# graphdeco-inria/editable-gaussian-reflections

Hardware: AMD Instinct MI355X
Metric: Mrays/s fwd+bwd @1080p, 1M Gaussians (higher is better)
Workload: dtype f32; 1 GPU; BASELINE config C: synthetic dense-init room+spheres cloud, HEADLINE variant = init (literal dense-init opacity 0.1 (config.py:44): Kc ~ 22 per ray, bounces mostly die), N=1000000, 1920x1080, one training iteration: export + update_bvh + forward + backward + grad import, num_bounces=2, jitter on, reference default config; variant=init, gaussians=1000000, width=1920, height=1080, parallelism=image tiles x1 + 1 all-reduce of the launch's [22N] gradients, team_help=product default (on)

## Files before the change

### editable-gaussian-reflections_amd/csrc/backward_chain.hpp

```cpp
#pragma once

constexpr int BOUNCE_QUEUE_FLOATS = 25 * EGR_WAVE;
static_assert(EGR_GT_STRIDE * EGR_GT_SLOTS >= BOUNCE_QUEUE_FLOATS, "the bounce queues must fit into the table");

template <int TEAM> struct BwdWave {
    int lane, wv;
    uint32_t *gt_keys;
    float *gt_vals;
    uint32_t *gt_claim;
    float4 *stage;
    BwdTeamShared<TEAM> &bteam;
    uint4 *bitems;
    float *bdl;
    float *bray;
    float exp_power;
    int num_bounces;
    float view_size;
    uint32_t bepoch;
    bool table_dirty;
};

struct BwdDiag {
    EGR_TIMES(unsigned long long bw_t0 = 0ull, bw_t1 = 0ull; uint32_t bw_rows0 = 0u;)
};
// ... 8 lines not shown

template <bool PRIMARY, bool BATCH, int TEAM>
EGR_DI RayGrads output_gradients(const DeviceView &v, const BwdWave<TEAM> &W, const ChainTask &task, const TaskGeom &tg, const StateRef &S, const int step,
                                 const uint32_t steps_done, const uint32_t nhits) {
    RayGrads g{mk3(0, 0, 0), mk3(0, 0, 0), mk3(0, 0, 0), 0.0f, 0.0f, mk3(0, 0, 0), mk3(0, 0, 1), mk3(0, 0, 0), mk3(0, 0, 0), mk3(0, 0, 0), 0.0f, 0.0f, 0.0f};
    if (nhits > 0) {
        const uint32_t pid = tg.pixel_id;
        const float third = 1.0f / 3.0f;
        if constexpr (PRIMARY) {
            f3 o_rgb = S.ld3(SF(0, S_RGB)), o_n = S.ld3(SF(0, S_NORMAL)), o_f0 = S.ld3(SF(0, S_F0));
            float o_depth = S.ld(SF(0, S_DEPTH)), o_rough = S.ld(SF(0, S_ROUGH));
            if constexpr (BATCH) {
                const size_t P = v.num_pixels;
                const uint32_t bframe = task.bframe;
                auto tgt = [&](int b, uint32_t ch, uint32_t c) { const float *p = v.batch_targets[b]; return p ? p[((size_t)bframe * ch + c) * P + pid] : 0.0f; };
                g.dL_rgb = mk3(third * sign1(o_rgb.x - tgt(0, 3, 0)), third * sign1(o_rgb.y - tgt(0, 3, 1)), third * sign1(o_rgb.z - tgt(0, 3, 2))) * *v.cfg.loss_weight_diffuse;
                g.dL_depth = sign1(o_depth - tgt(2, 1, 0)) * *v.cfg.loss_weight_depth;
                g.dL_n = mk3(third * sign1(o_n.x - tgt(3, 3, 0)), third * sign1(o_n.y - tgt(3, 3, 1)), third * sign1(o_n.z - tgt(3, 3, 2))) * *v.cfg.loss_weight_normal;
                g.dL_f0 = mk3(third * sign1(o_f0.x - tgt(5, 3, 0)), third * sign1(o_f0.y - tgt(5, 3, 1)), third * sign1(o_f0.z - tgt(5, 3, 2))) * *v.cfg.loss_weight_f0;
                g.dL_rough = sign1(o_rough - tgt(4, 1, 0)) * *v.cfg.loss_weight_roughness;
            } else {
                const bool planes = v.target_planes != 0u;
                const size_t cs = planes ? (size_t)v.num_pixels : (size_t)1;
                auto tgt = [&](int b, uint32_t ch, uint32_t c) { const float *p = v.batch_targets[b]; return p ? p[(size_t)pid * (planes ? 1u : ch) + c * cs] : 0.0f; };
                g.dL_rgb = mk3(third * sign1(o_rgb.x - tgt(0, 3, 0)), third * sign1(o_rgb.y - tgt(0, 3, 1)), third * sign1(o_rgb.z - tgt(0, 3, 2))) * *v.cfg.loss_weight_diffuse;
                g.dL_depth = sign1(o_depth - tgt(2, 1, 0)) * *v.cfg.loss_weight_depth;
                g.dL_n = mk3(third * sign1(o_n.x - tgt(3, 3, 0)), third * sign1(o_n.y - tgt(3, 3, 1)), third * sign1(o_n.z - tgt(3, 3, 2))) * *v.cfg.loss_weight_normal;
                g.dL_f0 = mk3(third * sign1(o_f0.x - tgt(5, 3, 0)), third * sign1(o_f0.y - tgt(5, 3, 1)), third * sign1(o_f0.z - tgt(5, 3, 2))) * *v.cfg.loss_weight_f0;
                g.dL_rough = sign1(o_rough - tgt(4, 1, 0)) * *v.cfg.loss_weight_roughness;
            }
            const PrimaryRay p = primary_ray<BATCH>(v, tg, task, W.view_size);
            g.ro = p.ro, g.rd = p.rd;
        } else {
            f3 spec = mk3(0, 0, 0);
            for (int j = 1; j < W.num_bounces + 1; j++)
                if ((uint32_t)j < steps_done) spec = spec + S.ld3(SF(j, S_RGB));
            f3 t_spec;
            if constexpr (BATCH) {
                const float *p = v.batch_targets[1];
                const size_t P = v.num_pixels, q = (size_t)task.bframe * 3 * P + pid;
                t_spec = p ? mk3(p[q], p[q + P], p[q + 2 * P]) : mk3(0, 0, 0);
            } else {
                const float *p = v.batch_targets[1];
                const size_t q = (size_t)pid * (v.target_planes ? 1u : 3u), cs = v.target_planes ? (size_t)v.num_pixels : (size_t)1;
                t_spec = p ? mk3(p[q], p[q + cs], p[q + 2 * cs]) : mk3(0, 0, 0);
            }
            float down = powf(1.0f - S.ld(SF(step - 1, S_ROUGH)), EGR_ROUGHNESS_DOWNWEIGHT_GRAD_POWER);
            g.dL_rgb = (mk3(third * sign1(spec.x - t_spec.x), third * sign1(spec.y - t_spec.y), third * sign1(spec.z - t_spec.z)) *
                        *v.cfg.loss_weight_specular) * down;
            g.dL_rgb = g.dL_rgb * S.ld3(SF(step - 1, S_THR));
            g.ro = S.ld3(SF(step - 1, S_NEXT_O));
            g.rd = S.ld3(SF(step - 1, S_NEXT_D));
        }
        g.rem_rgb = S.ld3(SF(step, S_REM_RGB)), g.rem_n = S.ld3(SF(step, S_REM_NORMAL)), g.rem_f0 = S.ld3(SF(step, S_REM_F0));
        g.rem_depth = S.ld(SF(step, S_REM_DEPTH)), g.rem_rough = S.ld(SF(step, S_REM_ROUGH));
        g.T_minus_Ttot = S.ld(SF(step, S_T)) - S.ld(SF(step, S_TTOT));
    }
    return g;
}

template <int TEAM> EGR_DI uint32_t bounce_hits(const DeviceView &v, BwdWave<TEAM> &W, const RayGrads &g, uint32_t blk, const uint32_t nhits, const uint32_t max_hits) {
    const int lane = W.lane, wv = W.wv;
    const float exp_power = W.exp_power;
    BwdTeamShared<TEAM> &bteam = W.bteam;
    uint4 *const bitems = W.bitems;
    float *const bdl = W.bdl, *const bray = W.bray;
    float4 *const stage = W.stage;
    const f3 dL_rgb = g.dL_rgb, ro = g.ro, rd = g.rd, rem_rgb = g.rem_rgb;
    const float T_minus_Ttot = g.T_minus_Ttot;
    uint32_t records = 0u;
    W.table_dirty = true;
    bdl[lane] = dL_rgb.x, bdl[EGR_WAVE + lane] = dL_rgb.y, bdl[2 * EGR_WAVE + lane] = dL_rgb.z;
    bray[lane] = ro.x, bray[EGR_WAVE + lane] = ro.y, bray[2 * EGR_WAVE + lane] = ro.z, bray[3 * EGR_WAVE + lane] = rd.x, bray[4 * EGR_WAVE + lane] = rd.y, bray[5 * EGR_WAVE + lane] = rd.z;
    f3 prev_rgb = mk3(0, 0, 0), w_rgb = mk3(0, 0, 0);
    const uint32_t nblocks = (max_hits + EGR_HIT_BLOCK_ROWS - 1) / EGR_HIT_BLOCK_ROWS;
    EGR_BWD_SYNC();
    for (uint32_t b = nblocks; b-- > 0;) {
        const float4 *rows = v.hit_arena + (size_t)blk * (EGR_HIT_BLOCK_ROWS + 1) * EGR_WAVE;
        for (int chunk = EGR_HIT_BLOCK_ROWS / 4 - 1; chunk >= 0; chunk--) {
            uint32_t nitems = 0u;
            float4 rec4[4], a04[4];
#pragma unroll
            for (int r4 = 0; r4 < 4; r4++) rec4[r4] = rows[(size_t)(1 + 4 * chunk + r4) * EGR_WAVE + lane];
#pragma unroll
            for (int r4 = 0; r4 < 4; r4++) a04[r4] = v.app[2 * ((b * EGR_HIT_BLOCK_ROWS + (uint32_t)(4 * chunk + r4)) < nhits ? f2u(rec4[r4].x) : 0u)];
#pragma unroll
            for (int r4 = 3; r4 >= 0; r4--) {
                const int row = 4 * chunk + r4;
                const uint32_t it = b * EGR_HIT_BLOCK_ROWS + (uint32_t)row;
                const bool act = it < nhits;
                float dL_dalpha = 0.0f, weight = 0.0f;
                uint32_t pos = 0u;
                if (act) {
                    const float4 rec = rec4[r4];
                    pos = f2u(rec.x);
                    const float alpha = rec.z, transmittance = rec.w;
                    weight = (float)((double)transmittance / (1.0 - (double)alpha) * (double)alpha);
                    const float4 a0 = a04[r4];
                    const f3 g_rgb = mk3(a0.x, a0.y, a0.z);
                    w_rgb = w_rgb + (g_rgb - prev_rgb) * transmittance;
                    prev_rgb = g_rgb;
                    const float one_m_alpha = 1.0f - alpha, r1ma = egr_rcp_refined(one_m_alpha);
                    const float tmp1 = egr_div_rn(1.0f, one_m_alpha, r1ma);
                    dL_dalpha += dot(w_rgb * tmp1, dL_rgb);
                    const float tmp2 = -egr_div_rn(T_minus_Ttot, one_m_alpha, r1ma);
                    dL_dalpha += tmp2 * dot(rem_rgb, dL_rgb);
                }
                const unsigned long long am = __ballot(act);
                if (act) bitems[nitems + __builtin_amdgcn_mbcnt_hi((uint32_t)(am >> 32), __builtin_amdgcn_mbcnt_lo((uint32_t)am, 0u))] = make_uint4((uint32_t)lane, f2u(dL_dalpha), pos, f2u(weight));
                nitems += (uint32_t)__popcll(am);
            }
            if (nitems == 0u) continue;
            EGR_BWD_SYNC();
            const uint32_t nbatch = (nitems + (uint32_t)EGR_WAVE - 1u) / (uint32_t)EGR_WAVE;
            if constexpr (TEAM > 1) {
                if (lane == 0) {
                    lds_poke(&bteam.finished[wv], 0u);
                    lds_poke(&bteam.nitems[wv], nitems);
                    W.bepoch = (W.bepoch + 1u) & 0xFFFu;
                    lds_poke(&bteam.ticket[wv], (W.bepoch << 20) | (nbatch << 10));
                }
                for (;;) {
                    uint32_t tk = 0u;
                    if (lane == 0) tk = atomicAdd(&bteam.ticket[wv], 1u);
                    tk = uniform_u32(tk);
                    const uint32_t bi = tk & 0x3FFu;
                    if (bi >= nbatch) break;
                    records += bounce_batch(v, exp_power, bitems, bdl, bray, bi * (uint32_t)EGR_WAVE, nitems, stage, lane);
                    if (lane == 0) atomicAdd(&bteam.finished[wv], 1u);
                }
                while (uniform_u32(lds_peek(&bteam.finished[wv])) < nbatch) __builtin_amdgcn_s_sleep(1);
            } else {
                for (uint32_t bi = 0; bi < nbatch; bi++) records += bounce_batch(v, exp_power, bitems, bdl, bray, bi * (uint32_t)EGR_WAVE, nitems, stage, lane);
            }
            EGR_BWD_SYNC();
        }
        blk = f2u(rows[0].x);
    }
    return records;
}

template <int TEAM> EGR_DI uint32_t primary_hits(const DeviceView &v, BwdWave<TEAM> &W, const RayGrads &g, uint32_t blk, const uint32_t nhits, const uint32_t max_hits) {
    const int lane = W.lane;
    uint32_t *const gt_keys = W.gt_keys, *const gt_claim = W.gt_claim;
    float *const gt_vals = W.gt_vals;
    float4 *const stage = W.stage;
    const f3 dL_rgb = g.dL_rgb, dL_n = g.dL_n, dL_f0 = g.dL_f0, ro = g.ro, rd = g.rd, rem_rgb = g.rem_rgb, rem_n = g.rem_n, rem_f0 = g.rem_f0;
    const float dL_depth = g.dL_depth, dL_rough = g.dL_rough, rem_depth = g.rem_depth, rem_rough = g.rem_rough, T_minus_Ttot = g.T_minus_Ttot;
    uint32_t records = 0u;
    f3 prev_rgb = mk3(0, 0, 0), w_rgb = mk3(0, 0, 0), prev_n = mk3(0, 0, 0), w_n = mk3(0, 0, 0), prev_f0 = mk3(0, 0, 0), w_f0 = mk3(0, 0, 0);
    float prev_rough = 0, w_rough = 0, prev_depth = 0, w_depth = 0;
    const uint32_t nblocks = (max_hits + EGR_HIT_BLOCK_ROWS - 1) / EGR_HIT_BLOCK_ROWS;
    EGR_STATS(unsigned long long bt_math = 0ull, bt_table = 0ull, bt_wide = 0ull, bt_rows = 0ull;)
    for (uint32_t b = nblocks; b-- > 0;) {
        const float4 *rows = v.hit_arena + (size_t)blk * (EGR_HIT_BLOCK_ROWS + 1) * EGR_WAVE;
        int pf_row = -1;
        float4 rec_pf = make_float4(0.f, 0.f, 0.f, 0.f);
        for (int row = EGR_HIT_BLOCK_ROWS - 1; row >= 0; row--) {
            const uint32_t it = b * EGR_HIT_BLOCK_ROWS + (uint32_t)row;
            if (it >= max_hits) continue;
            bool direct = false, want = false;
            uint32_t dpos = 0;
            float gx[EGR_GT_COMPS];
            EGR_STATS(const unsigned long long bt0 = __builtin_amdgcn_s_memtime(); unsigned long long bt1 = bt0; bt_rows++;)
            float4 rec_cur = rec_pf;
            const bool have_pf = pf_row == row;
            if (row > 0) {
                if (it <= nhits) rec_pf = rows[(size_t)row * EGR_WAVE + lane];
                pf_row = row - 1;
            }
            if (!have_pf) {
                if (it < nhits) rec_cur = rows[(size_t)(1 + row) * EGR_WAVE + lane];
#if defined(__HIP_DEVICE_COMPILE__)
                asm volatile("" ::"v"(rec_cur.x), "v"(rec_cur.y), "v"(rec_cur.z), "v"(rec_cur.w));
#endif
            }
            if (it < nhits) {
                const float4 rec = rec_cur;
                const uint32_t pos = f2u(rec.x);
                const float distance = rec.y, alpha = rec.z, transmittance = rec.w;
                const float4 a0 = v.app[2 * pos], a1 = v.app[2 * pos + 1], a2 = v.inst_w[4 * pos + 3];
                const f3 g_rgb = mk3(a0.x, a0.y, a0.z);
                const float weight = (float)((double)transmittance / (1.0 - (double)alpha) * (double)alpha);
                f3 d_rgb = (dL_rgb * weight);
                f3 d_n = dL_n * weight, d_f0 = dL_f0 * weight;
                float d_rough = dL_rough * weight;

                w_rgb = w_rgb + (g_rgb - prev_rgb) * transmittance;
                prev_rgb = g_rgb;
                {
                    f3 g_n = mk3(a0.w, a1.x, a1.y), g_f0 = mk3(a1.z, a1.w, a2.x);
                    w_n = w_n + (g_n - prev_n) * transmittance;
                    prev_n = g_n;
                    w_f0 = w_f0 + (g_f0 - prev_f0) * transmittance;
                    prev_f0 = g_f0;
                    w_rough += (a2.y - prev_rough) * transmittance;
                    prev_rough = a2.y;
                    w_depth += (distance - prev_depth) * transmittance;
                    prev_depth = distance;
                }
                float dL_dalpha = 0.0f;
                const float one_m_alpha = 1.0f - alpha, r1ma = egr_rcp_refined(one_m_alpha);
                const float tmp1 = egr_div_rn(1.0f, one_m_alpha, r1ma);
                dL_dalpha += dot(w_rgb * tmp1, dL_rgb);
                dL_dalpha += dot(w_n * tmp1, dL_n);
                dL_dalpha += dot(w_f0 * tmp1, dL_f0);
                dL_dalpha += (w_rough * tmp1) * dL_rough;
                dL_dalpha += (w_depth * tmp1) * dL_depth;
                const float tmp2 = -egr_div_rn(T_minus_Ttot, one_m_alpha, r1ma);
                dL_dalpha += tmp2 * dot(rem_rgb, dL_rgb);
                dL_dalpha += tmp2 * dot(rem_n, dL_n);
                dL_dalpha += tmp2 * dot(rem_f0, dL_f0);
                dL_dalpha += tmp2 * (rem_rough * dL_rough);
                dL_dalpha += tmp2 * (rem_depth * dL_depth);

                hit_geometry_fn(v, W.exp_power, pos, a2, ro, rd, dL_dalpha, gx);
                gx[PC_RGB] = d_rgb.x, gx[PC_RGB + 1] = d_rgb.y, gx[PC_RGB + 2] = d_rgb.z, gx[PC_WEIGHT] = weight;
                gx[PC_NORMAL] = d_n.x, gx[PC_NORMAL + 1] = d_n.y, gx[PC_NORMAL + 2] = d_n.z;
                gx[PC_F0] = d_f0.x, gx[PC_F0 + 1] = d_f0.y, gx[PC_F0 + 2] = d_f0.z, gx[PC_ROUGH] = d_rough;
                EGR_STATS(bt1 = __builtin_amdgcn_s_memtime();)
                dpos = pos;
                want = primary_presum(pos, gx, lane);
            }
            direct = primary_table_add(v, want, dpos, gx, gt_keys, gt_vals, gt_claim, stage, lane, records);
            EGR_STATS(const unsigned long long bt2 = __builtin_amdgcn_s_memtime(); bt_math += bt1 - bt0; bt_table += bt2 - bt1;)
            if (__ballot(direct) != 0ull) {
                float lo[EGR_REC0_COMPS], hi[EGR_REC1_COMPS];
#pragma unroll
                for (int c = 0; c < EGR_REC0_COMPS; c++) lo[c] = gx[c];
#pragma unroll
                for (int c = 0; c < EGR_REC1_COMPS; c++) hi[c] = gx[EGR_REC0_COMPS + c];
                wide_add_wave<EGR_REC0_CELL>(v, direct, dpos, lo, stage);
                wide_add_wave<EGR_REC1_CELL>(v, direct, dpos, hi, stage);
                records += 2u * (uint32_t)__popcll(__ballot(direct));
            }
            EGR_STATS(bt_wide += __builtin_amdgcn_s_memtime() - bt2;)
        }
        blk = f2u(rows[0].x);
    }
    EGR_STATS(const unsigned long long bt3 = __builtin_amdgcn_s_memtime();)
    records += grad_table_flush(v, gt_keys, gt_vals, stage, lane);
    EGR_STATS(if (lane == 0) {
        unsigned long long *d = diag64(v.control, DG_BWD_MATH_CYC);
        atomicAdd(d, bt_math), atomicAdd(d + 1, bt_table), atomicAdd(d + 2, bt_wide), atomicAdd(d + 3, __builtin_amdgcn_s_memtime() - bt3), atomicAdd(d + 4, bt_rows);
    })
    return records;
}

template <bool PRIMARY, int TEAM, bool BATCH> EGR_DI uint32_t backward_step(const DeviceView &v, BwdWave<TEAM> &W, const uint32_t tq, const int step, BwdDiag &D) {
    const int lane = W.lane;
    const uint32_t tqo = v.bwd_order[tq];
    const uint32_t blk = v.task_last_block[(size_t)step * (BATCH ? v.num_tasks * v.batch_frames : v.num_tasks) + tqo];
    if (blk == 0xFFFFFFFFu) return 0u;
    const ChainTask task = decode_task<BATCH>(v, tqo);
    const TaskGeom tg = task_geom(v, task.tb, lane);
    const StateRef S = state_of(v, task.tq, lane);
    const uint32_t steps_done = tg.inside ? f2u(S.ld(F_STEPS)) : 0u;
    const uint32_t nhits = (tg.inside && (uint32_t)step < steps_done && blk != 0xFFFFFFFFu) ? f2u(S.ld(SF(step, S_NHITS))) : 0u;
    const uint32_t max_hits = wave_max_u32(nhits);
    if (max_hits == 0) return 0u;
    EGR_TIMES_IS(8, if (PRIMARY) D.bw_rows0 = max_hits;)
    const RayGrads g = output_gradients<PRIMARY, BATCH>(v, W, task, tg, S, step, steps_done, nhits);
    if constexpr (PRIMARY) return primary_hits(v, W, g, blk, nhits, max_hits);
    else return bounce_hits(v, W, g, blk, nhits, max_hits);
}

template <int TEAM, bool BATCH> EGR_DI void backward_chain(const DeviceView v) {
    const int lane = threadIdx.x & (EGR_WAVE - 1);
    const int wv = __builtin_amdgcn_readfirstlane((int)(threadIdx.x >> 6));
    __shared__ uint32_t gt_keys_all[TEAM][EGR_GT_SLOTS];
    __shared__ __attribute__((aligned(16))) float gt_vals_all[TEAM][EGR_GT_STRIDE * EGR_GT_SLOTS];
    __shared__ uint32_t gt_claim_all[TEAM][EGR_GT_SLOTS];
    __shared__ float4 stage_all[TEAM][4 * EGR_WAVE];
    __shared__ BwdTeamShared<TEAM> bteam;
    if (threadIdx.x == 0) bteam.done = 0u;
    if (threadIdx.x < TEAM) bteam.ticket[threadIdx.x] = 0u, bteam.nitems[threadIdx.x] = 0u, bteam.finished[threadIdx.x] = 0u;
    uint32_t *const gt_keys = gt_keys_all[wv];
    float *const gt_vals = gt_vals_all[wv];
    for (int s = lane; s < EGR_GT_SLOTS; s += EGR_WAVE) gt_keys[s] = EGR_GT_EMPTY;
    for (int s = lane; s < EGR_GT_STRIDE * EGR_GT_SLOTS; s += EGR_WAVE) gt_vals[s] = 0.0f;
    __syncthreads();
    const float exp_power = *v.cfg.exp_power;
    const int num_bounces = min(*v.cfg.num_bounces, EGR_MAX_BOUNCES);
    const float view_size = BATCH ? 0.0f : tanf(*v.cam.vertical_fov_radians / 2.0f);
    BwdWave<TEAM> W{lane, wv, gt_keys, gt_vals, gt_claim_all[wv], stage_all[wv], bteam, reinterpret_cast<uint4 *>(gt_vals), gt_vals + 16 * EGR_WAVE, gt_vals + 19 * EGR_WAVE,
                    exp_power, num_bounces, view_size, 0u, false};
    uint32_t cur_q = blockIdx.x & 7u;
    uint32_t records = 0u;

    for (;;) {
        const uint32_t tq = wave_next_task(v.queues + 8 * EGR_QUEUE_STRIDE, BATCH ? v.num_tasks * v.batch_frames : v.num_tasks, cur_q, lane);
        if (tq == 0xFFFFFFFFu) break;
        BwdDiag D;
        EGR_TIMES_IS(8, D.bw_t0 = __builtin_amdgcn_s_memrealtime();)
        W.table_dirty = false;
        records += backward_step<true, TEAM, BATCH>(v, W, tq, 0, D);
        EGR_TIMES_IS(8, D.bw_t1 = __builtin_amdgcn_s_memrealtime();)
        for (int step = num_bounces; step >= 1; step--) records += backward_step<false, TEAM, BATCH>(v, W, tq, step, D);
        if (W.table_dirty) {
            EGR_BWD_SYNC();
            for (int s = lane; s < BOUNCE_QUEUE_FLOATS; s += EGR_WAVE) gt_vals[s] = 0.0f;
            EGR_BWD_SYNC();
        }
        EGR_TIMES_IS(8,
            const unsigned long long bw_t2 = __builtin_amdgcn_s_memrealtime();
            const TaskGeom btg = task_geom(v, decode_task<BATCH>(v, v.bwd_order[tq]).tb, lane);
            if (btg.inside) {
                if (lane == 0) v.stats.num_traversed_per_pixel[btg.pixel_id] = EGR_STAMP31(D.bw_t0), v.stats.num_accumulated_per_pixel[btg.pixel_id] = EGR_STAMP31(bw_t2);
                if (lane == 1) v.stats.num_traversed_per_pixel[btg.pixel_id] = EGR_STAMP31(D.bw_t1), v.stats.num_accumulated_per_pixel[btg.pixel_id] = (int32_t)D.bw_rows0;
            })
    }
    if constexpr (TEAM > 1) {
        if (lane == 0) atomicAdd(&bteam.done, 1u);
        records += bwd_team_help<TEAM>(v, exp_power, bteam, gt_vals_all, W.stage, wv, lane);
    }
    if (lane == 0 && records) atomicAdd(v.control + CW_BUCKET_RECORDS, records);
}
```

### editable-gaussian-reflections_amd/csrc/egr_diag.hpp

```cpp
#pragma once
#include <stdio.h>

#include "egr_internal.hpp"
#ifdef EGR_TRAVERSAL_STATS
#define EGR_STATS(...) __VA_ARGS__
#else
#define EGR_STATS(...)
#endif
#ifdef EGR_TASK_TIMES
#define EGR_TIMES(...) __VA_ARGS__
#else
#define EGR_TIMES(...)
#endif
#define EGR_TIMES_IS(n, ...) EGR_TIMES(if (EGR_TASK_TIMES == (n)) { __VA_ARGS__ })
#if defined(EGR_TRAVERSAL_STATS) || defined(EGR_TASK_TIMES)
#define EGR_WALK_STATS 1
#define EGR_WALK(...) __VA_ARGS__
#else
#define EGR_WALK(...)
#endif
#define EGR_STAMP31(t) ((int32_t)((t) & 0x7FFFFFFFull))

enum DiagSlot : int {
    DG_BEGIN = 32,
    DG_VISITS = 32, DG_LEAF_HITS = 34, DG_WALK_ITERS = 36, DG_EVAL_ROUNDS = 38, DG_TRAVERSAL_CYC = 40, DG_COMPOSITE_CYC = 42, DG_LEAF_EVAL_CYC = 44, DG_BWD_MATH_CYC = 46 , DG_CLASS_STRIDE = 24,
    DG_EPILOGUE_CYC = 80, DG_CHAIN_CYC = 82, DG_FILTER_CYC = 84, DG_FILTER_LEAVES = 86, DG_COMP_SCAN_CYC = 88 ,
    DG_LIST_HIST = 98 , DG_TEAM_OFFERS = 124, DG_TEAM_HELPED = 125, DG_TEAM_HELP_ITERS = 126, DG_TEAM_TALL = 127,
    DG_STEP_EXIT = 112,
    DG_END = 128
};
static_assert((int)DG_BEGIN > (int)CW_LIFE_LAUNCHES && (int)DG_END <= (int)CW_HIT_BUMP, "the diagnostic words lie between the counters and the bump allocators");
static_assert(CW_HIT_BUMP % 32 == 0 && CW_EXT_BUMP % 32 == 0 && CW_EXT_BUMP >= CW_HIT_BUMP + 32 && CW_COUNT >= CW_EXT_BUMP + 32, "DESIGN.md: a word many waves update with atomics starts a 128-B line that holds nothing else");
enum DiagKind : uint8_t { DK_COUNT, DK_CYCLES  };
struct DiagEntry { int slot, bits; DiagKind kind; bool per_class; const char *group, *label; };
constexpr DiagEntry EGR_DIAG_TABLE[] = {
    {DG_VISITS, 64, DK_COUNT, true, "", "lane node visits"},
    {DG_LEAF_HITS, 64, DK_COUNT, true, "", "lane leaf-box hits"},
    {DG_WALK_ITERS, 64, DK_COUNT, true, "", "wave inner iterations"},
    {DG_EVAL_ROUNDS, 64, DK_COUNT, true, "", "wave outer rounds"},
    {DG_TRAVERSAL_CYC, 64, DK_CYCLES, true, "", "traversal"},
    {DG_COMPOSITE_CYC, 64, DK_CYCLES, true, "", "composite"},
    {DG_LEAF_EVAL_CYC, 64, DK_CYCLES, true, "", "of the traversal: leaf evaluation (frustum walk)"},
    {DG_BWD_MATH_CYC, 64, DK_CYCLES, true, "backward ", "per-hit math"},
    {DG_BWD_MATH_CYC + 2, 64, DK_CYCLES, true, "backward ", "neighbour combine + LDS table"},
    {DG_BWD_MATH_CYC + 4, 64, DK_CYCLES, true, "backward ", "wide adds"},
    {DG_BWD_MATH_CYC + 6, 64, DK_CYCLES, true, "backward ", "table flush"},
    {DG_BWD_MATH_CYC + 8, 64, DK_COUNT, true, "backward ", "hit rows"},
    {DG_EPILOGUE_CYC, 64, DK_CYCLES, false, "forward chain", "step epilogues"},
    {DG_CHAIN_CYC, 64, DK_CYCLES, false, "forward chain", "whole chains (task pull to end)"},
    {DG_FILTER_CYC, 64, DK_CYCLES, false, "primary leaf filter", "sphere / pyramid test"},
    {DG_FILTER_LEAVES, 64, DK_COUNT, false, "primary leaf filter", "leaves before the test"},
    {DG_COMP_SCAN_CYC, 64, DK_CYCLES, false, "primary composite", "selection scans"},
    {DG_COMP_SCAN_CYC + 2, 64, DK_CYCLES, false, "primary composite", "arena block"},
    {DG_COMP_SCAN_CYC + 4, 64, DK_CYCLES, false, "primary composite", "alpha / record fetch"},
    {DG_COMP_SCAN_CYC + 6, 64, DK_CYCLES, false, "primary composite", "pass 1"},
    {DG_COMP_SCAN_CYC + 8, 64, DK_CYCLES, false, "primary composite", "appearance pass"},
    {DG_LIST_HIST, 32, DK_COUNT, false, "primary lists", "tiles by their longest candidate list: <=16"},
    {DG_LIST_HIST + 1, 32, DK_COUNT, false, "primary lists", "<=24"},
    {DG_LIST_HIST + 2, 32, DK_COUNT, false, "primary lists", "<=32"},
    {DG_LIST_HIST + 3, 32, DK_COUNT, false, "primary lists", "<=40"},
    {DG_LIST_HIST + 4, 32, DK_COUNT, false, "primary lists", "<=48"},
    {DG_LIST_HIST + 5, 32, DK_COUNT, false, "primary lists", "<=64"},
    {DG_LIST_HIST + 6, 32, DK_COUNT, false, "primary lists", "longer"},
    {DG_TEAM_OFFERS, 32, DK_COUNT, false, "team", "offers made"},
    {DG_TEAM_HELPED, 32, DK_COUNT, false, "team", "offers walked by helpers"},
    {DG_TEAM_HELP_ITERS, 32, DK_COUNT, false, "team", "their walk iterations"},
    {DG_TEAM_TALL, 32, DK_COUNT, false, "team", "owner walk iterations that left >= EGR_DONATE_MIN pairs on the stack"},
};
constexpr bool egr_diag_layout_ok() {
    int end = DG_BEGIN;
    for (const DiagEntry &d : EGR_DIAG_TABLE) {
        const int lo = d.per_class ? DG_BEGIN : DG_BEGIN + 2 * DG_CLASS_STRIDE, hi = d.per_class ? DG_BEGIN + DG_CLASS_STRIDE : DG_END, e = d.slot + d.bits / 32;
        if (d.slot < end || d.slot < lo || e > hi || (d.bits == 64 && d.slot % 2 != 0) || (e > DG_STEP_EXIT && d.slot < DG_STEP_EXIT + 12)) return false;
        end = e;
    }
    return true;
}
static_assert(egr_diag_layout_ok(), "diagnostic slots: inside [DG_BEGIN, DG_END), disjoint, 64-bit ones 8-byte aligned");

inline void egr_diag_print(const uint32_t *w) {
    const int n = (int)(sizeof(EGR_DIAG_TABLE) / sizeof(EGR_DIAG_TABLE[0]));
    for (int i = 0, j; i < n; i = j) {
        const DiagEntry &g = EGR_DIAG_TABLE[i];
        for (j = i + 1; j < n && __builtin_strcmp(EGR_DIAG_TABLE[j].group, g.group) == 0; j++) {}
        for (int k = 0; k <= (g.per_class ? 1 : 0); k++) {
            fprintf(stderr, "[egr stats %s%s]", g.group, !g.per_class ? "" : k ? "bounce" : "primary");
            for (int e = i; e < j; e++) {
                const int s = EGR_DIAG_TABLE[e].slot + k * DG_CLASS_STRIDE;
                const unsigned long long x = EGR_DIAG_TABLE[e].bits == 64 ? (unsigned long long)w[s] | ((unsigned long long)w[s + 1] << 32) : w[s];
                fprintf(stderr, "%s %s %llu%s", e > i ? "," : "", EGR_DIAG_TABLE[e].label, x, EGR_DIAG_TABLE[e].kind == DK_CYCLES ? " wave-cycles" : "");
            }
            fputc('\n', stderr);
        }
    }
}

#if defined(EGR_TRAVERSAL_STATS) && defined(__HIPCC__)
__device__ __forceinline__ unsigned long long *diag64(uint32_t *control, int slot, bool bounce = false) { return reinterpret_cast<unsigned long long *>(control + slot + (bounce ? DG_CLASS_STRIDE : 0)); }
#endif
```

### editable-gaussian-reflections_amd/csrc/trace.hip

```cpp
#include <algorithm>
#include <cstdio>
#include <cstdlib>
#include <type_traits>
#include <utility>
#include <vector>

#define EGR_CONTRACT_AFTER_EPILOGUE
#include "egr_diag.hpp"
#include "egr_epilogue.hpp"

#ifndef EGR_GPOP
#define EGR_GPOP 5
#endif
#define EGR_WALK_MAX_LEAVES (8 * EGR_GPOP * EGR_WIDTH)
#define EGR_LBUF (64 + 2 * EGR_WALK_MAX_LEAVES)
#ifndef EGR_FPOP
#define EGR_FPOP 2
#endif
#ifndef EGR_PSTK
#define EGR_PSTK 512
#endif

namespace {

// ... 535 lines not shown
    const int t = threadIdx.x;
    reset_launch_words(v, t);
    reset_chunk_words(v, t);
    if (t == 0) {
        *v.meta.grads_enabled = grads ? 1 : 0;
        *v.meta.total_num_calls += 1;
    }
}
__global__ void k_epilogue(DeviceView v, int grads) {
    if (threadIdx.x == 0) {
        if (*v.cfg.accumulate_samples) *v.fb.accumulated_sample_count += 1;
        count_lifetime(v, 1u);
    }
}
__global__ void __launch_bounds__(256) k_live(DeviceView v, int grads) {
    uint32_t i = blockIdx.x * 256 + threadIdx.x;
    if (i >= v.n) return;
    const egr_gaussians &g = v.g;
    float o = sigmoid_act(g.opacity[i]);
    float sigma = compute_scaling_factor(o, *v.cfg.alpha_threshold, *v.cfg.exp_power);
    const size_t pos = v.pos_of_gid[i];
    float4 *app = v.app + 2 * pos;
    app[0] = make_float4(relu_act(g.rgb[3 * i]), relu_act(g.rgb[3 * i + 1]), relu_act(g.rgb[3 * i + 2]), g.normal[3 * i]);
    app[1] = make_float4(g.normal[3 * i + 1], g.normal[3 * i + 2], clip01_act(g.f0[3 * i]), clip01_act(g.f0[3 * i + 1]));
    v.inst_w[4 * pos + 3] = make_float4(clip01_act(g.f0[3 * i + 2]), clip01_act(g.roughness[i]), o, sigma);
    if (grads) {
        float4 *im = v.inst_m + 4 * (size_t)i;
        im[0].w = expf(g.scale[3 * i]), im[1].w = expf(g.scale[3 * i + 1]), im[2].w = expf(g.scale[3 * i + 2]);
        im[3] = reinterpret_cast<const float4 *>(g.rotation)[i];
    }
}

#ifndef EGR_ARENA_CHUNK
#define EGR_ARENA_CHUNK 8
#endif
#ifndef EGR_FWD_WAVES
#define EGR_FWD_WAVES 4
#endif
template <bool GRADS, bool CUBE, int TEAM> __global__ void __launch_bounds__(EGR_WAVE * TEAM) __attribute__((amdgpu_waves_per_eu(EGR_FWD_WAVES, EGR_FWD_WAVES))) k_forward_chain(DeviceView v) {
    constexpr bool BATCH = false, OBJ = false;
    [[maybe_unused]] const ObjectQuery oq{};
    [[maybe_unused]] float *const oacc = nullptr;
#include "forward_chain.inc"
}
template <bool CUBE, int TEAM> __global__ void __launch_bounds__(EGR_WAVE * TEAM) __attribute__((amdgpu_waves_per_eu(EGR_FWD_WAVES, EGR_FWD_WAVES))) k_forward_batch(DeviceView v) {
    constexpr bool GRADS = false, BATCH = true, OBJ = false;
    [[maybe_unused]] const ObjectQuery oq{};
    [[maybe_unused]] float *const oacc = nullptr;
#include "forward_chain.inc"
}
template <bool CUBE, int TEAM> __global__ void __launch_bounds__(EGR_WAVE * TEAM) __attribute__((amdgpu_waves_per_eu(EGR_FWD_WAVES, EGR_FWD_WAVES))) k_forward_batch_grads(DeviceView v) {
    constexpr bool GRADS = true, BATCH = true, OBJ = false;
    [[maybe_unused]] const ObjectQuery oq{};
    [[maybe_unused]] float *const oacc = nullptr;
#include "forward_chain.inc"
}
#ifndef EGR_OBJ_WAVES
#define EGR_OBJ_WAVES EGR_FWD_WAVES
#endif
#ifndef EGR_OBJ_MIN_SUMS
#define EGR_OBJ_MIN_SUMS 1
#endif
extern __shared__ float egr_object_sums[];
__global__ void __launch_bounds__(EGR_WAVE) __attribute__((amdgpu_waves_per_eu(EGR_OBJ_WAVES, EGR_OBJ_WAVES))) k_forward_objects(DeviceView v, ObjectQuery oq) {
    constexpr bool GRADS = false, BATCH = true, OBJ = true, CUBE = false;
    constexpr int TEAM = 1;
    float *const oacc = egr_object_sums;
#include "forward_chain.inc"
}
__global__ void __launch_bounds__(256) k_object_bits(DeviceView v, const uint32_t *__restrict__ row_bits, ObjectBitList bits, uint32_t num_bits, uint32_t *__restrict__ pos_bits) {
    const uint32_t p = blockIdx.x * 256u + threadIdx.x;
    if (p >= v.n) return;
    const uint32_t w = row_bits[v.gid_of_pos[p]];
    uint32_t out = 0u;
    for (uint32_t j = 0; j < num_bits; j++) out |= ((w >> bits.bit[j]) & 1u) << j;
    pos_bits[p] = out;
}
__global__ void k_objects_prologue(DeviceView v) {
    reset_launch_words(v, threadIdx.x);
    reset_chunk_words(v, threadIdx.x);
}

#ifndef EGR_GT_SLOTS
#define EGR_GT_SLOTS 80
#endif
#define EGR_GT_COMPS 21
#define EGR_GT_STRIDE 21
#define EGR_GT_EMPTY 0xFFFFFFFFu
enum : int { GC_OPA = 0, GC_MEAN = 1, GC_RGB = 4, GC_WEIGHT = 7, GC_Q = 8, GC_NORMAL = 16, GC_F0 = 19, GC_ROUGH = 22 };
enum : int { PC_OPA = 0, PC_MEAN = 1, PC_RGB = 4, PC_WEIGHT = 7, PC_Q = 8, PC_NORMAL = 14, PC_F0 = 17, PC_ROUGH = 20 };
#define EGR_REC0_CELL 0
#define EGR_REC0_COMPS 14
#define EGR_REC1_CELL 16
#define EGR_REC1_COMPS 7
static_assert(EGR_REC0_COMPS + EGR_REC1_COMPS == EGR_GT_COMPS && PC_NORMAL == EGR_REC0_COMPS && GC_NORMAL == EGR_REC1_CELL, "the table's components are the two records, in order");
#define EGR_ROW_STRIDE 32
#define EGR_BWD_SYNC() wave_sync()

template <int CELL, int N> EGR_DI void wide_add_wave(const DeviceView &v, bool ok, uint32_t pos, const float (&r)[N], float4 *stage) {
    static_assert(N >= 1 && N <= 15, "a record is its row index and up to 15 values: 16 lanes");
    static_assert(CELL >= 0 && CELL / 16 == (CELL + N - 1) / 16 && CELL + N <= EGR_ROW_STRIDE, "a record's cells lie in ONE 64-B segment of the row");
    const int lane = threadIdx.x & (EGR_WAVE - 1);
    const uint32_t cell = (uint32_t)CELL + (uint32_t)((lane & 15) - 1);
    if (ok) {
        auto rv = [&](int i) { return i < N ? r[i < N ? i : 0] : 0.0f; };
        stage[4 * lane + 0] = make_float4(u2f(pos), rv(0), rv(1), rv(2));
        if (N > 3) stage[4 * lane + 1] = make_float4(rv(3), rv(4), rv(5), rv(6));
        if (N > 7) stage[4 * lane + 2] = make_float4(rv(7), rv(8), rv(9), rv(10));
        if (N > 11) stage[4 * lane + 3] = make_float4(rv(11), rv(12), rv(13), rv(14));
    }
    const unsigned long long okm = __ballot(ok);
    EGR_BWD_SYNC();
    const float *sf = reinterpret_cast<const float *>(stage);
#pragma unroll 4
    for (int pass = 0; pass < 16; pass++) {
        const int src = 4 * pass + (lane >> 4), c = lane & 15;
        if (((okm >> (4 * pass)) & 0xFull) == 0ull) continue;
        const float x = sf[16 * src + c];
        const uint32_t p = f2u(sf[16 * src]);
        if (((okm >> src) & 1ull) && c != 0 && c <= N && x != 0.0f) atomicAdd(v.grad_rows + (size_t)p * EGR_ROW_STRIDE + cell, x);
    }
    EGR_BWD_SYNC();
}

EGR_DI uint32_t grad_table_flush(const DeviceView &v, uint32_t *gt_keys, float *gt_vals, float4 *stage, int lane) {
    uint32_t sent = 0u;
    EGR_BWD_SYNC();
    for (int s0 = 0; s0 < EGR_GT_SLOTS; s0 += EGR_WAVE) {
        const int s = min(s0 + lane, EGR_GT_SLOTS - 1);
        const bool in_table = s0 + lane < EGR_GT_SLOTS;
        const uint32_t pos = in_table ? gt_keys[s] : EGR_GT_EMPTY;
        const bool valid = pos != EGR_GT_EMPTY;
        if (in_table) gt_keys[s] = EGR_GT_EMPTY;
        float lo[EGR_REC0_COMPS], hi[EGR_REC1_COMPS];
#pragma unroll
        for (int c = 0; c < EGR_REC0_COMPS; c++) {
            lo[c] = valid ? gt_vals[s * EGR_GT_STRIDE + c] : 0.0f;
            if (valid) gt_vals[s * EGR_GT_STRIDE + c] = 0.0f;
        }
#pragma unroll
        for (int c = 0; c < EGR_REC1_COMPS; c++) {
            hi[c] = valid ? gt_vals[s * EGR_GT_STRIDE + EGR_REC0_COMPS + c] : 0.0f;
            if (valid) gt_vals[s * EGR_GT_STRIDE + EGR_REC0_COMPS + c] = 0.0f;
        }
        if (__ballot(valid) == 0ull) continue;
        wide_add_wave<EGR_REC0_CELL>(v, valid, pos, lo, stage);
        wide_add_wave<EGR_REC1_CELL>(v, valid, pos, hi, stage);
        sent += 2u * (uint32_t)__popcll(__ballot(valid));
    }
    EGR_BWD_SYNC();
    return sent;
}

EGR_DI bool primary_presum(const uint32_t pos, float (&gx)[EGR_GT_COMPS], const int lane) {
#pragma clang fp contract(off)
    bool mine = true;
    {
        const unsigned long long em = __ballot(true);
#define EGR_FETCH_DPP(x, ctrl) __builtin_amdgcn_update_dpp(0, (int)(x), ctrl, 0xF, 0xF, false)
#define EGR_COMBINE(d, FETCH, arg)                                                                            \
    {                                                                                                          \
        const bool pact = ((em >> ((uint32_t)lane ^ (d))) & 1ull) != 0ull;                                     \
        const uint32_t ppos = (uint32_t)FETCH(pos, arg), pmine = (uint32_t)FETCH(mine ? 1 : 0, arg);           \
        const bool same = pact && pmine != 0u && mine && ppos == pos;                                          \
        const bool take = same && ((uint32_t)lane & (d)) == 0u;                                                \
        _Pragma("unroll") for (int c = 0; c < EGR_GT_COMPS; c++) {                                             \
            const float s = gx[c] + __int_as_float(FETCH(__float_as_int(gx[c]), arg));                         \
            gx[c] = take ? s : gx[c];                                                                          \
        }                                                                                                      \
        if (same && !take) mine = false;                                                                       \
    }
        EGR_COMBINE(1u, EGR_FETCH_DPP, 0xB1)
        EGR_COMBINE(8u, EGR_FETCH_DPP, 0x128)
#undef EGR_COMBINE
#undef EGR_FETCH_DPP
    }
    return mine;
}
EGR_DI bool primary_table_add(const DeviceView &v, const bool want, const uint32_t pos, const float (&gx)[EGR_GT_COMPS], uint32_t *gt_keys, float *gt_vals, uint32_t *gt_claim, float4 *stage,
                              const int lane, uint32_t &records) {
    bool found = false;
    uint32_t slot = 0u;
    auto probe = [&]() {
        slot = ((((pos * 2654435761u) >> 16) * (uint32_t)EGR_GT_SLOTS) >> 16);
        found = false;
#pragma unroll 1
        for (int pr = 0; pr < (want ? 8 : 0); pr++) {
            uint32_t key = *reinterpret_cast<volatile uint32_t *>(&gt_keys[slot]);
            if (key == EGR_GT_EMPTY) key = atomicCAS(&gt_keys[slot], EGR_GT_EMPTY, pos), key = key == EGR_GT_EMPTY ? pos : key;
            if (key == pos) { found = true; break; }
            slot = slot + 1u == (uint32_t)EGR_GT_SLOTS ? 0u : slot + 1u;
        }
    };
    probe();
    if (__ballot(want && !found) != 0ull) {
        records += grad_table_flush(v, gt_keys, gt_vals, stage, lane);
        probe();
    }
    bool pending = found;
    while (__ballot(pending) != 0ull) {
        if (pending) gt_claim[slot] = (uint32_t)lane;
        EGR_BWD_SYNC();
        const bool win = pending && gt_claim[slot] == (uint32_t)lane;
        if (win) {
            float *cell = gt_vals + slot * EGR_GT_STRIDE;
            float cur[EGR_GT_COMPS];
#pragma unroll
            for (int c = 0; c < EGR_GT_COMPS; c++) cur[c] = cell[c];
#pragma unroll
            for (int c = 0; c < EGR_GT_COMPS; c++) cell[c] = cur[c] + gx[c];
            pending = false;
        }
        EGR_BWD_SYNC();
    }
    return want && !found;
}

struct ChainVec { double x, y, z; };
EGR_DI void scale_rot_chain(const float4 &M0, const float4 &M1, const float4 &M2, const float4 &qu, const float sigma, const float eps, const ChainVec &dl2w0, const ChainVec &dl2w1,
                            const ChainVec &dl2w2, double (&d_scale)[3], double (&d_rot)[4]) {
    using T = double;
    const T scaling_factor = sigma, eps_scale_grad = eps;
    const ChainVec scaling = {T(M0.w), T(M1.w), T(M2.w)};
    const ChainVec den = {scaling.x * scaling_factor + eps_scale_grad, scaling.y * scaling_factor + eps_scale_grad, scaling.z * scaling_factor + eps_scale_grad};
    auto div3 = [&](const float4 &m) { return ChainVec{T(m.x) / den.x, T(m.y) / den.y, T(m.z) / den.z}; };
    const ChainVec rot_0 = div3(M0), rot_1 = div3(M1), rot_2 = div3(M2);
    d_scale[0] = (dl2w0.x * rot_0.x + dl2w1.x * rot_1.x + dl2w2.x * rot_2.x) * scaling.x;
    d_scale[1] = (dl2w0.y * rot_0.y + dl2w1.y * rot_1.y + dl2w2.y * rot_2.y) * scaling.y;
    d_scale[2] = (dl2w0.z * rot_0.z + dl2w1.z * rot_1.z + dl2w2.z * rot_2.z) * scaling.z;
    auto mul3 = [](const ChainVec &a, const ChainVec &b) { return ChainVec{a.x * b.x, a.y * b.y, a.z * b.z}; };
    const ChainVec dr0 = mul3(dl2w0, scaling), dr1 = mul3(dl2w1, scaling), dr2 = mul3(dl2w2, scaling);
    const T qr = qu.x, qx = qu.y, qy = qu.z, qz = qu.w;
    const T qn = sqrt(qr * qr + qx * qx + qy * qy + qz * qz);
    const T r = qr / qn, x = qx / qn, y = qy / qn, z = qz / qn;
    const T dL_dr = T(2) * x * (dr2.y - dr1.z) + T(2) * y * (dr0.z - dr2.x) + T(2) * z * (dr1.x - dr0.y);
    const T dL_dx = T(-4) * x * (dr1.y + dr2.z) + T(2) * y * (dr0.y + dr1.x) + T(2) * z * (dr0.z + dr2.x) + T(2) * r * (dr2.y - dr1.z);
    const T dL_dy = T(2) * x * (dr0.y + dr1.x) - T(4) * y * (dr0.x + dr2.z) + T(2) * z * (dr1.z + dr2.y) + T(2) * r * (dr0.z - dr2.x);
    const T dL_dz = T(2) * x * (dr0.z + dr2.x) + T(2) * y * (dr1.z + dr2.y) - T(4) * z * (dr0.x + dr1.y) + T(2) * r * (dr1.x - dr0.y);
    const T dd = dL_dr * qr + dL_dx * qx + dL_dy * qy + dL_dz * qz;
    const T qn3 = qn * qn * qn;
    const T inv3 = T(1) / qn3, inv1 = T(1) / qn;
    d_rot[0] = dd * -qr * inv3 + dL_dr * inv1, d_rot[1] = dd * -qx * inv3 + dL_dx * inv1;
    d_rot[2] = dd * -qy * inv3 + dL_dy * inv1, d_rot[3] = dd * -qz * inv3 + dL_dz * inv1;
}

template <class GX> EGR_DI void hit_geometry_fn(const DeviceView &v, const float exp_power, uint32_t pos, const float4 &a2, const f3 &ro, const f3 &rd, float dL_dalpha, GX &gx) {
    const float opacity = a2.z, scaling_factor = a2.w;
    const float4 W0 = v.inst_w[4 * pos], W1 = v.inst_w[4 * pos + 1], W2 = v.inst_w[4 * pos + 2];
    f3 lo, ld, dhat, u;
    float t_unused;
    bool behind_unused, outside_unused;
    candidate_geometry(W0, W1, W2, ro, rd, lo, ld, dhat, t_unused, u, behind_unused, outside_unused);
    const f3 local_hit = u * scaling_factor;
    const float sq_norm = dot(local_hit, local_hit);
    const float gaussval = egr_gaussian_sq(sq_norm, exp_power);

    float d_opacity = EGR_MAX_ALPHA * dL_dalpha * gaussval;
    d_opacity = d_opacity * opacity * (1.0f - opacity);
    const float dL_dgaussval = EGR_MAX_ALPHA * dL_dalpha * opacity;
    const float dL_dsq_norm = gaussval * pow_exp_m1(sq_norm, exp_power);
    const f3 dL_dx_local = (-local_hit * dL_dsq_norm) * dL_dgaussval;
    const f3 dL_dx_world = mk3(dot(mk3(W0.x, W1.x, W2.x), dL_dx_local), dot(mk3(W0.y, W1.y, W2.y), dL_dx_local),
                               dot(mk3(W0.z, W1.z, W2.z), dL_dx_local)) * scaling_factor;
    const f3 d_mean = -dL_dx_world;
    gx[PC_OPA] = d_opacity, gx[PC_MEAN] = d_mean.x, gx[PC_MEAN + 1] = d_mean.y, gx[PC_MEAN + 2] = d_mean.z;
    const f3 ql = -dL_dx_local * scaling_factor;
    gx[PC_Q] = ql.x * local_hit.x, gx[PC_Q + 1] = ql.x * local_hit.y, gx[PC_Q + 2] = ql.x * local_hit.z;
    gx[PC_Q + 3] = ql.y * local_hit.y, gx[PC_Q + 4] = ql.y * local_hit.z, gx[PC_Q + 5] = ql.z * local_hit.z;
}

EGR_DI uint32_t bounce_batch(const DeviceView &v, const float exp_power, const uint4 *bitems, const float *bdl, const float *bray, uint32_t i0, uint32_t nitems, float4 *stage, int lane) {
    static_assert(PC_OPA == GC_OPA && PC_MEAN == GC_MEAN && PC_RGB == GC_RGB && PC_WEIGHT == GC_WEIGHT && PC_Q == GC_Q && GC_Q + 6 == EGR_REC0_COMPS, "components 0-13 of a hit are segment 0 of the row");
    const bool valid = i0 + (uint32_t)lane < nitems;
    uint32_t dpos = 0;
    float gx[EGR_REC0_COMPS];
#pragma unroll
    for (int c = 0; c < EGR_REC0_COMPS; c++) gx[c] = 0.0f;
    if (valid) {
        const uint4 item = bitems[i0 + (uint32_t)lane];
        const uint32_t ray = item.x, pos = item.z;
        const float weight = u2f(item.w);
        const float4 a2 = v.inst_w[4 * pos + 3];
        const f3 iro = mk3(bray[ray], bray[EGR_WAVE + ray], bray[2 * EGR_WAVE + ray]), ird = mk3(bray[3 * EGR_WAVE + ray], bray[4 * EGR_WAVE + ray], bray[5 * EGR_WAVE + ray]);
        hit_geometry_fn(v, exp_power, pos, a2, iro, ird, u2f(item.y), gx);
        gx[GC_RGB] = bdl[ray] * weight, gx[GC_RGB + 1] = bdl[EGR_WAVE + ray] * weight, gx[GC_RGB + 2] = bdl[2 * EGR_WAVE + ray] * weight;
        gx[GC_WEIGHT] = weight;
        dpos = pos;
    }
    wide_add_wave<EGR_REC0_CELL>(v, valid, dpos, gx, stage);
    return (uint32_t)__popcll(__ballot(valid));
}

#ifndef EGR_BWD_TEAM
#define EGR_BWD_TEAM 4
#endif
template <int TEAM> struct BwdTeamShared {
    uint32_t done;
    uint32_t ticket[TEAM], nitems[TEAM], finished[TEAM];
};

#ifndef EGR_BWD_WAVES
#define EGR_BWD_WAVES 3
#endif
#ifndef EGR_ORDER_BUCKETS
#define EGR_ORDER_BUCKETS 16
#endif
#ifndef EGR_ORDER_SHIFT
#define EGR_ORDER_SHIFT 7
#endif
__global__ void __launch_bounds__(256) k_order_backward(DeviceView v) {
    __shared__ uint32_t cnt[EGR_ORDER_BUCKETS][256 + 1];
    const uint32_t chunk = ((v.num_tasks + 7u) / 8u + 3u) & ~3u, q = blockIdx.x;
    const uint32_t beg = q * chunk, end = min(beg + chunk, v.num_tasks);
    if (beg >= end) return;
    const uint32_t t = threadIdx.x, n = end - beg, per = (n + 255u) / 256u;
    const uint32_t i0 = min(t * per, n), i1 = min(i0 + per, n);
    auto bucket = [](uint32_t cost) { return (uint32_t)EGR_ORDER_BUCKETS - 1u - min(cost >> EGR_ORDER_SHIFT, (uint32_t)EGR_ORDER_BUCKETS - 1u); };
    for (int b = 0; b < EGR_ORDER_BUCKETS; b++) cnt[b][t] = 0u;
    for (uint32_t i = i0; i < i1; i++) cnt[bucket(v.task_cost[beg + i])][t]++;
    __syncthreads();
    if (t < (uint32_t)EGR_ORDER_BUCKETS) {
        uint32_t acc = 0u;
        for (int j = 0; j < 256; j++) {
            const uint32_t c = cnt[t][j];
            cnt[t][j] = acc, acc += c;
        }
        cnt[t][256] = acc;
    }
    __syncthreads();
    uint32_t start[EGR_ORDER_BUCKETS];
    uint32_t acc = 0u;
#pragma unroll
    for (int b = 0; b < EGR_ORDER_BUCKETS; b++) start[b] = acc + cnt[b][t], acc += cnt[b][256];
    for (uint32_t i = i0; i < i1; i++) {
        const uint32_t bk = bucket(v.task_cost[beg + i]);
        uint32_t at = 0u;
#pragma unroll
        for (int b = 0; b < EGR_ORDER_BUCKETS; b++)
            if ((uint32_t)b == bk) at = start[b]++;
        v.bwd_order[beg + at] = beg + i;
    }
}

template <int TEAM> EGR_DI uint32_t bwd_team_help(const DeviceView &v, const float exp_power, BwdTeamShared<TEAM> &bteam, float (*gt_vals_all)[EGR_GT_STRIDE * EGR_GT_SLOTS],
                                                  float4 *stage, const int wv, const int lane) {
    uint32_t records = 0u;
    while (uniform_u32(lds_peek(&bteam.done)) < (uint32_t)TEAM) {
        bool any = false;
        for (int dlt = 1; dlt < TEAM; dlt++) {
            const int w = (wv + dlt) % TEAM;
            const uint32_t peek = uniform_u32(lds_peek(&bteam.ticket[w]));
            if ((peek & 0x3FFu) >= ((peek >> 10) & 0x3FFu)) continue;
            uint32_t tk = 0u;
            if (lane == 0) tk = atomicAdd(&bteam.ticket[w], 1u);
            tk = uniform_u32(tk);
            const uint32_t bi = tk & 0x3FFu, nbatch = (tk >> 10) & 0x3FFu;
            if (bi >= nbatch) continue;
            const uint32_t nitems = uniform_u32(lds_peek(&bteam.nitems[w]));
            const uint4 *bitems = reinterpret_cast<const uint4 *>(gt_vals_all[w]);
            records += bounce_batch(v, exp_power, bitems, gt_vals_all[w] + 16 * EGR_WAVE, gt_vals_all[w] + 19 * EGR_WAVE, bi * (uint32_t)EGR_WAVE, nitems, stage, lane);
            if (lane == 0) atomicAdd(&bteam.finished[w], 1u);
            any = true;
        }
        if (!any) __builtin_amdgcn_s_sleep(2);
    }
    return records;
}
// ... 765 lines not shown
```

Baseline: 477.0 Mrays/s.

## Merge duplicate-key gradient adds via atomicExch chains and pointer jumping

Replaces the DPP pre-sum and the claim-and-retry loop in the primary backward gradient table with a per-slot linked list. Each lane atomically exchanges its id into the slot's claim word. Lanes then reduce along the chain with ds_bpermute pointer jumping, and only the leader writes the summed gradient to LDS. This removes the serialized claim/sync rounds when many lanes in a wave hit the same Gaussian, at the cost of extra bpermute traffic across all gradient components on each jump step. It also adds stats-only counters and initializes the claim array to empty.

Result: faster. 493.3 Mrays/s (median of 6 runs) (+3.4%).

```diff
diff --git a/editable-gaussian-reflections_amd/csrc/backward_chain.hpp b/editable-gaussian-reflections_amd/csrc/backward_chain.hpp
--- a/editable-gaussian-reflections_amd/csrc/backward_chain.hpp
+++ b/editable-gaussian-reflections_amd/csrc/backward_chain.hpp
@@ -184,6 +184,7 @@
     float prev_rough = 0, w_rough = 0, prev_depth = 0, w_depth = 0;
     const uint32_t nblocks = (max_hits + EGR_HIT_BLOCK_ROWS - 1) / EGR_HIT_BLOCK_ROWS;
     EGR_STATS(unsigned long long bt_math = 0ull, bt_table = 0ull, bt_wide = 0ull, bt_rows = 0ull;)
+    EGR_STATS(unsigned long long bt_lanes = 0ull, bt_steps = 0ull, bt_leaders = 0ull;)
     for (uint32_t b = nblocks; b-- > 0;) {
         const float4 *rows = v.hit_arena + (size_t)blk * (EGR_HIT_BLOCK_ROWS + 1) * EGR_WAVE;
         int pf_row = -1;
@@ -252,9 +253,11 @@
                 gx[PC_F0] = d_f0.x, gx[PC_F0 + 1] = d_f0.y, gx[PC_F0 + 2] = d_f0.z, gx[PC_ROUGH] = d_rough;
                 EGR_STATS(bt1 = __builtin_amdgcn_s_memtime();)
                 dpos = pos;
-                want = primary_presum(pos, gx, lane);
-            }
-            direct = primary_table_add(v, want, dpos, gx, gt_keys, gt_vals, gt_claim, stage, lane, records);
+                want = true;
+            }
+            uint32_t jump_steps, row_leaders;
+            direct = primary_table_add(v, want, dpos, gx, gt_keys, gt_vals, gt_claim, stage, lane, records, jump_steps, row_leaders);
+            EGR_STATS(bt_lanes += (unsigned long long)__popcll(__ballot(want)); bt_steps += jump_steps; bt_leaders += row_leaders;)
             EGR_STATS(const unsigned long long bt2 = __builtin_amdgcn_s_memtime(); bt_math += bt1 - bt0; bt_table += bt2 - bt1;)
             if (__ballot(direct) != 0ull) {
                 float lo[EGR_REC0_COMPS], hi[EGR_REC1_COMPS];
@@ -275,6 +278,8 @@
     EGR_STATS(if (lane == 0) {
         unsigned long long *d = diag64(v.control, DG_BWD_MATH_CYC);
         atomicAdd(d, bt_math), atomicAdd(d + 1, bt_table), atomicAdd(d + 2, bt_wide), atomicAdd(d + 3, __builtin_amdgcn_s_memtime() - bt3), atomicAdd(d + 4, bt_rows);
+        unsigned long long *r = diag64(v.control, DG_BWD_ROW_GROUPS);
+        atomicAdd(r, bt_lanes), atomicAdd(r + 1, bt_steps), atomicAdd(r + 2, bt_leaders);
     })
     return records;
 }
@@ -309,7 +314,7 @@
     if (threadIdx.x < TEAM) bteam.ticket[threadIdx.x] = 0u, bteam.nitems[threadIdx.x] = 0u, bteam.finished[threadIdx.x] = 0u;
     uint32_t *const gt_keys = gt_keys_all[wv];
     float *const gt_vals = gt_vals_all[wv];
-    for (int s = lane; s < EGR_GT_SLOTS; s += EGR_WAVE) gt_keys[s] = EGR_GT_EMPTY;
+    for (int s = lane; s < EGR_GT_SLOTS; s += EGR_WAVE) gt_keys[s] = EGR_GT_EMPTY, gt_claim_all[wv][s] = EGR_GT_EMPTY;
     for (int s = lane; s < EGR_GT_STRIDE * EGR_GT_SLOTS; s += EGR_WAVE) gt_vals[s] = 0.0f;
     __syncthreads();
     const float exp_power = *v.cfg.exp_power;
diff --git a/editable-gaussian-reflections_amd/csrc/egr_diag.hpp b/editable-gaussian-reflections_amd/csrc/egr_diag.hpp
--- a/editable-gaussian-reflections_amd/csrc/egr_diag.hpp
+++ b/editable-gaussian-reflections_amd/csrc/egr_diag.hpp
@@ -25,7 +25,7 @@
     DG_BEGIN = 32,
     DG_VISITS = 32, DG_LEAF_HITS = 34, DG_WALK_ITERS = 36, DG_EVAL_ROUNDS = 38, DG_TRAVERSAL_CYC = 40, DG_COMPOSITE_CYC = 42, DG_LEAF_EVAL_CYC = 44, DG_BWD_MATH_CYC = 46 , DG_CLASS_STRIDE = 24,
     DG_EPILOGUE_CYC = 80, DG_CHAIN_CYC = 82, DG_FILTER_CYC = 84, DG_FILTER_LEAVES = 86, DG_COMP_SCAN_CYC = 88 ,
-    DG_LIST_HIST = 98 , DG_TEAM_OFFERS = 124, DG_TEAM_HELPED = 125, DG_TEAM_HELP_ITERS = 126, DG_TEAM_TALL = 127,
+    DG_LIST_HIST = 98 , DG_BWD_ROW_GROUPS = 106 , DG_TEAM_OFFERS = 124, DG_TEAM_HELPED = 125, DG_TEAM_HELP_ITERS = 126, DG_TEAM_TALL = 127,
     DG_STEP_EXIT = 112,
     DG_END = 128
 };
@@ -62,6 +62,9 @@
     {DG_LIST_HIST + 4, 32, DK_COUNT, false, "primary lists", "<=48"},
     {DG_LIST_HIST + 5, 32, DK_COUNT, false, "primary lists", "<=64"},
     {DG_LIST_HIST + 6, 32, DK_COUNT, false, "primary lists", "longer"},
+    {DG_BWD_ROW_GROUPS, 64, DK_COUNT, false, "backward primary", "lanes with a hit"},
+    {DG_BWD_ROW_GROUPS + 2, 64, DK_COUNT, false, "backward primary", "pointer-jumping steps"},
+    {DG_BWD_ROW_GROUPS + 4, 64, DK_COUNT, false, "backward primary", "leaders"},
     {DG_TEAM_OFFERS, 32, DK_COUNT, false, "team", "offers made"},
     {DG_TEAM_HELPED, 32, DK_COUNT, false, "team", "offers walked by helpers"},
     {DG_TEAM_HELP_ITERS, 32, DK_COUNT, false, "team", "their walk iterations"},
diff --git a/editable-gaussian-reflections_amd/csrc/trace.hip b/editable-gaussian-reflections_amd/csrc/trace.hip
--- a/editable-gaussian-reflections_amd/csrc/trace.hip
+++ b/editable-gaussian-reflections_amd/csrc/trace.hip
@@ -711,33 +711,9 @@
     return sent;
 }
 
-EGR_DI bool primary_presum(const uint32_t pos, float (&gx)[EGR_GT_COMPS], const int lane) {
+EGR_DI bool primary_table_add(const DeviceView &v, const bool want, const uint32_t pos, float (&gx)[EGR_GT_COMPS], uint32_t *gt_keys, float *gt_vals, uint32_t *gt_claim, float4 *stage,
+                              const int lane, uint32_t &records, uint32_t &steps, uint32_t &leaders) {
 #pragma clang fp contract(off)
-    bool mine = true;
-    {
-        const unsigned long long em = __ballot(true);
-#define EGR_FETCH_DPP(x, ctrl) __builtin_amdgcn_update_dpp(0, (int)(x), ctrl, 0xF, 0xF, false)
-#define EGR_COMBINE(d, FETCH, arg)                                                                            \
-    {                                                                                                          \
-        const bool pact = ((em >> ((uint32_t)lane ^ (d))) & 1ull) != 0ull;                                     \
-        const uint32_t ppos = (uint32_t)FETCH(pos, arg), pmine = (uint32_t)FETCH(mine ? 1 : 0, arg);           \
-        const bool same = pact && pmine != 0u && mine && ppos == pos;                                          \
-        const bool take = same && ((uint32_t)lane & (d)) == 0u;                                                \
-        _Pragma("unroll") for (int c = 0; c < EGR_GT_COMPS; c++) {                                             \
-            const float s = gx[c] + __int_as_float(FETCH(__float_as_int(gx[c]), arg));                         \
-            gx[c] = take ? s : gx[c];                                                                          \
-        }                                                                                                      \
-        if (same && !take) mine = false;                                                                       \
-    }
-        EGR_COMBINE(1u, EGR_FETCH_DPP, 0xB1)
-        EGR_COMBINE(8u, EGR_FETCH_DPP, 0x128)
-#undef EGR_COMBINE
-#undef EGR_FETCH_DPP
-    }
-    return mine;
-}
-EGR_DI bool primary_table_add(const DeviceView &v, const bool want, const uint32_t pos, const float (&gx)[EGR_GT_COMPS], uint32_t *gt_keys, float *gt_vals, uint32_t *gt_claim, float4 *stage,
-                              const int lane, uint32_t &records) {
     bool found = false;
     uint32_t slot = 0u;
     auto probe = [&]() {
@@ -745,7 +721,7 @@
         found = false;
 #pragma unroll 1
         for (int pr = 0; pr < (want ? 8 : 0); pr++) {
-            uint32_t key = *reinterpret_cast<volatile uint32_t *>(&gt_keys[slot]);
+            uint32_t key = lds_peek(&gt_keys[slot]);
             if (key == EGR_GT_EMPTY) key = atomicCAS(&gt_keys[slot], EGR_GT_EMPTY, pos), key = key == EGR_GT_EMPTY ? pos : key;
             if (key == pos) { found = true; break; }
             slot = slot + 1u == (uint32_t)EGR_GT_SLOTS ? 0u : slot + 1u;
@@ -756,22 +732,42 @@
         records += grad_table_flush(v, gt_keys, gt_vals, stage, lane);
         probe();
     }
-    bool pending = found;
-    while (__ballot(pending) != 0ull) {
-        if (pending) gt_claim[slot] = (uint32_t)lane;
-        EGR_BWD_SYNC();
-        const bool win = pending && gt_claim[slot] == (uint32_t)lane;
-        if (win) {
-            float *cell = gt_vals + slot * EGR_GT_STRIDE;
-            float cur[EGR_GT_COMPS];
-#pragma unroll
-            for (int c = 0; c < EGR_GT_COMPS; c++) cur[c] = cell[c];
-#pragma unroll
-            for (int c = 0; c < EGR_GT_COMPS; c++) cell[c] = cur[c] + gx[c];
-            pending = false;
-        }
-        EGR_BWD_SYNC();
-    }
+    uint32_t prev = (uint32_t)lane;
+    if (found) {
+        const uint32_t before = atomicExch(&gt_claim[slot], (uint32_t)lane);
+        prev = before == EGR_GT_EMPTY ? (uint32_t)lane : before;
+    }
+    EGR_BWD_SYNC();
+    const bool leader = found && lds_peek(&gt_claim[slot]) == (uint32_t)lane;
+    if (leader) lds_poke(&gt_claim[slot], EGR_GT_EMPTY);
+    steps = 0u, leaders = (uint32_t)__popcll(__ballot(leader));
+    unsigned long long more = __ballot(prev != (uint32_t)lane);
+#pragma unroll 1
+    while (more != 0ull) {
+        const bool take = prev != (uint32_t)lane;
+        const int from = (int)(prev << 2);
+        float o[EGR_GT_COMPS];
+#pragma unroll
+        for (int c = 0; c < EGR_GT_COMPS; c++) o[c] = __int_as_float(__builtin_amdgcn_ds_bpermute(from, __float_as_int(gx[c])));
+        const uint32_t p2 = (uint32_t)__builtin_amdgcn_ds_bpermute(from, (int)prev);
+#pragma unroll
+        for (int c = 0; c < EGR_GT_COMPS; c++) {
+            const float s = gx[c] + o[c];
+            gx[c] = take ? s : gx[c];
+        }
+        prev = p2 == prev ? (uint32_t)lane : p2;
+        more = __ballot(prev != (uint32_t)lane);
+        steps++;
+    }
+    if (leader) {
+        float *cell = gt_vals + slot * EGR_GT_STRIDE;
+        float cur[EGR_GT_COMPS];
+#pragma unroll
+        for (int c = 0; c < EGR_GT_COMPS; c++) cur[c] = cell[c];
+#pragma unroll
+        for (int c = 0; c < EGR_GT_COMPS; c++) cell[c] = cur[c] + gx[c];
+    }
+    EGR_BWD_SYNC();
     return want && !found;
 }
 
```
